# nanless/universal-speech-enhancement

Measured on AMD Instinct MI355X. Metric: spectrogram-frames/sec through 30-step PC sampler, 24 kHz, higher is better.
Workload: dtype bf16; 1 GPU; configs[1]: NCSN++ Large score net, batch=8x4 s utterances per GPU, 30-step PC sampler (reverse_diffusion + langevin x1, snr 0.5, 60 NFE), bf16, hipGraph=on; global_batch=8, frames_per_utt=601, padded_frames_per_utt=640, n_freq=512, N=30, nfe=60, parallelism=utterance-sharded x1

## Files before the change

universal_speech_enhancement_amd/csrc/use_conv_v2.hip:

```cpp
#include "use_kernels.h"
#include "use_device.h"

#include <cstdio>
#include <cstdlib>

namespace use {

constexpr int V2_T = 16;
constexpr int V2_HE = V2_T + 2;
constexpr int V2_HALO = V2_HE * V2_HE;
constexpr int V2_BN = 128;

template <typename TIN, bool ACT>
DEVI uint4 v2_transform(const uint4 raw, const unsigned mask, const float (&ca)[16 / sizeof(TIN)],
                        const float (&cb)[16 / sizeof(TIN)]) {
    constexpr int VEC = 16 / sizeof(TIN);
    float v[VEC];
    Vec16<TIN>::load(reinterpret_cast<const TIN*>(&raw), v);
#pragma unroll
    for (int k = 0; k < VEC; ++k) {
        v[k] = fmaf(v[k], ca[k], cb[k]);
        if (ACT) {
            if (sizeof(TIN) == 4) v[k] = v[k] / (1.0f + expf(-v[k]));
            else v[k] = v[k] * __builtin_amdgcn_rcpf(1.0f + __builtin_amdgcn_exp2f(v[k] * -1.44269504088896341f));
        }
    }
    uint4 o = Vec16<TIN>::pack(v);
    o.x &= mask; o.y &= mask; o.z &= mask; o.w &= mask;
    return o;
}

template <typename TIN, typename TOUT, int CK, bool ACT>
__global__ __launch_bounds__(512) void conv_v2_kernel(ConvArgs p) {
    typedef Mfma<TIN> MF;
    constexpr int VEC = 16 / sizeof(TIN);
    constexpr int PARTS = CK / VEC;
    constexpr int ROWB = CK * (int)sizeof(TIN) + 16;
    constexpr int BN = V2_BN, WM = 4, WN = 2, MW = 64, NW = 64, TM = 2, TN = 2;
    constexpr int KSTEPS = CK / MF::KM;
    constexpr int HPITCH = (V2_HE * ROWB / 16 + 15) / 16 * 16 * 16;
    constexpr int HALO_BYTES = V2_HE * HPITCH, W_BYTES = BN * ROWB;
    constexpr int MAIN_BYTES = 2 * HALO_BYTES + 2 * W_BYTES;
    constexpr int NPIECE = V2_HALO * PARTS;
    constexpr int PIECE_ITERS = (NPIECE + 511) / 512;
    static_assert(PARTS == 8 && 512 % PARTS == 0 && PIECE_ITERS <= 8, "v2 staging assumes 128-byte chunk rows");

    extern __shared__ __attribute__((aligned(16))) char smem[];
    const int tid = threadIdx.x, lane = tid & 63, wave = tid >> 6;
    const int wm = wave / WN, wn = wave % WN;
    const int b = blockIdx.z;
    int tile = blockIdx.x;
    if ((gridDim.x & 7) == 0) tile = (blockIdx.x & 7) * (gridDim.x >> 3) + (blockIdx.x >> 3);
    const int tiles_x = (p.W + V2_T - 1) / V2_T;
    const int ty0 = (tile / tiles_x) * V2_T, tx0 = (tile % tiles_x) * V2_T;
    const int n0 = blockIdx.y * BN;
    const int Ctot = p.C0 + p.C1;
    const int nchunks = Ctot / CK;
    const int XCtot = p.XC0 + p.XC1;
    const int nchunks2 = XCtot / CK;
    const int part = tid & (PARTS - 1);

    float addv[2];
#pragma unroll
    for (int j = 0; j < 2; ++j) {
        const int co = n0 + wn * 64 + j * 32 + (lane & 31);
        float add = 0.f;
// ... 35 lines not shown
    for (int i = 0; i < TM; ++i) {
        const int m = wm * MW + i * 32 + (lane & 31);
        a_base[i] = (m >> 4) * HPITCH + (m & 15) * ROWB + (lane >> 5) * MF::KPL * (int)sizeof(TIN);
    }
#pragma unroll
    for (int j = 0; j < TN; ++j)
        b_base[j] = 2 * HALO_BYTES + (wn * NW + j * 32 + (lane & 31)) * ROWB + (lane >> 5) * MF::KPL * (int)sizeof(TIN);

    int ppix[PIECE_ITERS], pdst[PIECE_ITERS]; unsigned pmask[PIECE_ITERS];
#pragma unroll
    for (int j = 0; j < PIECE_ITERS; ++j) {
        const int idx = j * 512 + tid;
        const int pix = idx / PARTS;
        const int hy = pix / V2_HE, hx = pix - hy * V2_HE;
        const int gy = ty0 + hy - 1, gx = tx0 + hx - 1;
        const bool inb = idx < NPIECE && gy >= 0 && gy < p.H && gx >= 0 && gx < p.W;
        ppix[j] = inb ? gy * p.W + gx : 0;
        pmask[j] = inb ? 0xffffffffu : 0u;
        pdst[j] = idx < NPIECE ? hy * HPITCH + hx * ROWB + part * 16 : -1;
    }
    const int dummy_off = MAIN_BYTES + tid * 16;
    constexpr int COEF_OFF = MAIN_BYTES + 512 * 16;
    float2* const coef_lds = reinterpret_cast<float2*>(smem + COEF_OFF);
    float ca[VEC], cb[VEC];
    auto load_coef = [&](int chunk) {
        const float2* cf = coef_lds + chunk * CK + part * VEC;
#pragma unroll
        for (int k = 0; k < VEC; ++k) { const float2 v = cf[k]; ca[k] = v.x; cb[k] = v.y; }
    };
    auto buf_ld = [&](const void* base, unsigned voff, unsigned soff) -> uint4 {
        const __amdgpu_buffer_rsrc_t rs = __builtin_amdgcn_make_buffer_rsrc(const_cast<void*>(base), 0, 0x7fffffff, 0x00020000);
        return __builtin_bit_cast(uint4, __builtin_amdgcn_raw_buffer_load_b128(rs, voff, soff, 0));
    };
    auto src_ld0 = [&](int chunk, int pixoff) -> uint4 {
        const int c_glob = chunk * CK;
        const TIN* src; int Cs, c_loc;
        if (c_glob < p.C0) { src = (const TIN*)p.src0; Cs = p.C0; c_loc = c_glob; }
        else               { src = (const TIN*)p.src1; Cs = p.C1; c_loc = c_glob - p.C0; }
        const unsigned voff = (unsigned)pixoff * (unsigned)(Cs * (int)sizeof(TIN)) + (unsigned)(part * 16);
        return buf_ld(src + (size_t)b * p.H * p.W * Cs, voff, (unsigned)(c_loc * (int)sizeof(TIN)));
    };
    auto load_piece1 = [&](int chunk2, int q, uint4& raw) -> unsigned {
        const int pix = (q * 512 + tid) / PARTS;
        const int gy = ty0 + (pix >> 4), gx = tx0 + (pix & 15);
        const bool inb = gy < p.H && gx < p.W;
        const int c_glob = chunk2 * CK;
        const TIN* src; int Cs, c_loc;
        if (c_glob < p.XC0) { src = (const TIN*)p.x0; Cs = p.XC0; c_loc = c_glob; }
        else                { src = (const TIN*)p.x1; Cs = p.XC1; c_loc = c_glob - p.XC0; }
        const size_t pixoff = inb ? (size_t)(b * p.H + gy) * p.W + gx : 0;
        raw = *reinterpret_cast<const uint4*>(src + pixoff * Cs + c_loc + part * VEC);
        return inb ? 0xffffffffu : 0u;
    };
    auto piece1_dst = [&](int q, int hb) -> int {
        const int pix = (q * 512 + tid) / PARTS;
        return hb * HALO_BYTES + ((pix >> 4) + 1) * HPITCH + ((pix & 15) + 1) * ROWB + part * 16;
    };

    const int wrow0 = tid / PARTS, wrow1 = (tid + 512) / PARTS;
    const unsigned wo0 = wrow0 * 9 * Ctot + part * VEC, wo1 = wrow1 * 9 * Ctot + part * VEC;
    const unsigned wob0 = wo0 * (unsigned)sizeof(TIN), wob1 = wo1 * (unsigned)sizeof(TIN);
    const int wdst0 = 2 * HALO_BYTES + wrow0 * ROWB + part * 16, wdst1 = 2 * HALO_BYTES + wrow1 * ROWB + part * 16;
    const TIN* const wseg0 = (const TIN*)p.w + (size_t)n0 * 9 * Ctot;
#define V2_LOAD_W(CC, TT, R0, R1)                                                                                    \
    {                                                                                                                \
        const int cw_ = (TT) > 8 ? (CC) + 1 : (CC);                                                                  \
        const int tw_ = (TT) > 8 ? (TT)-9 : (TT);                                                                    \
        if (cw_ < nchunks) {                                                                                         \
            const unsigned so_ = (unsigned)(tw_ * Ctot + cw_ * CK) * (unsigned)sizeof(TIN);                          \
            R0 = buf_ld(wseg0, wob0, so_); R1 = buf_ld(wseg0, wob1, so_);                                            \
        }                                                                                                            \
    }
#define V2_STORE_W(BUF, R0, R1)                                                                     \
    {                                                                                               \
        *reinterpret_cast<uint4*>(smem + (BUF)*W_BYTES + wdst0) = R0;                               \
        *reinterpret_cast<uint4*>(smem + (BUF)*W_BYTES + wdst1) = R1;                               \
    }

    uint4 wa0 = make_uint4(0, 0, 0, 0), wa1 = wa0;
    {
        uint4 w00 = wa0, w01 = wa0, raw[PIECE_ITERS];
        V2_LOAD_W(0, 0, w00, w01);
        V2_LOAD_W(0, 1, wa0, wa1);
#pragma unroll
        for (int j = 0; j < PIECE_ITERS; ++j) raw[j] = src_ld0(0, ppix[j]);
        gn_fill_table(coef_lds, p, b, Ctot, tid, 512);
        __syncthreads();
        load_coef(0);
        V2_STORE_W(0, w00, w01);
#pragma unroll
        for (int j = 0; j < PIECE_ITERS; ++j)
            *reinterpret_cast<uint4*>(smem + (pdst[j] >= 0 ? pdst[j] : dummy_off)) = v2_transform<TIN, ACT>(raw[j], pmask[j], ca, cb);
    }

    V2_STAMP(2)
    typename MF::frag af[KSTEPS][TM], bf[KSTEPS][TN];
    uint4 hL = wa0, hT = wa0, t0 = wa0;
#define V2_LDS(CC, T)                                                                                                \
    {                                                                                                                \
        const int cc_ = (CC);                                                                                        \
        const int par_ = cc_ & 1;                             \
        const bool next_ = cc_ + 1 < nchunks;                                                                        \
        V2_STAMPF(100 + (T))                                                                                          \
        {                                                                                                            \
            const char* ha_ = smem + par_ * HALO_BYTES + ((T) / 3) * HPITCH + ((T) % 3) * ROWB;                      \
            const char* wbuf_ = smem + (par_ ^ ((T)&1)) * W_BYTES;                                                   \
            _Pragma("unroll") for (int kk = 0; kk < KSTEPS; ++kk) {                                                  \
                _Pragma("unroll") for (int i = 0; i < TM; ++i) af[kk][i] = MF::ld(ha_ + a_base[i] + kk * MF::KM * (int)sizeof(TIN)); \
                _Pragma("unroll") for (int j = 0; j < TN; ++j) bf[kk][j] = MF::ld(wbuf_ + b_base[j] + kk * MF::KM * (int)sizeof(TIN)); \
            }                                                                                                        \
        }                                                                                                            \
        __builtin_amdgcn_sched_barrier(0);                                                                           \
        V2_STAMPF(500 + (T))                                                                                          \
        if ((T) >= 2 && (T) < PIECE_ITERS + 2 && next_) {                                                            \
            constexpr int k_ = (T) >= 2 && (T) < PIECE_ITERS + 2 ? (T)-2 : 0;                                        \
            *reinterpret_cast<uint4*>(smem + (pdst[k_] >= 0 ? (par_ ^ 1) * HALO_BYTES + pdst[k_] : dummy_off)) = t0;  \
        }                                                                                                            \
        if ((T) < 8 || next_) V2_STORE_W((par_ ^ ((T)&1)) ^ 1, wa0, wa1);                                            \
        V2_STAMPF(600 + (T))                                                                                          \
        if ((T) >= 1 && (T) < PIECE_ITERS + 1) {                                                                     \
             \
             \
            hT = hL;                                                                                                 \
            asm volatile("" : "+v"(hT.x), "+v"(hT.y), "+v"(hT.z), "+v"(hT.w));                                       \
        }                                                                                                            \
        if ((T) < PIECE_ITERS && next_) {                                                                            \
            if ((T) == 0) load_coef(cc_ + 1);                                                                        \
            constexpr int k_ = (T) < PIECE_ITERS ? (T) : 0;                                                          \
            hL = src_ld0(cc_ + 1, ppix[k_]);                                                                           \
        }                                                                                                            \
        V2_LOAD_W(cc_, (T) + 2, wa0, wa1);                                                                           \
        V2_STAMPF(200 + (T))                                                                                          \
    }
#define V2_MFMA(CC, T)                                                                                               \
    {                                                                                                                \
        V2_STAMPF(300 + (T))                                                                                          \
        _Pragma("unroll") for (int kk = 0; kk < KSTEPS; ++kk)                                                        \
            _Pragma("unroll") for (int i = 0; i < TM; ++i)                                                           \
                _Pragma("unroll") for (int j = 0; j < TN; ++j) acc[i][j] = MF::mma(af[kk][i], bf[kk][j], acc[i][j]);  \
        if ((T) >= 1 && (T) < PIECE_ITERS + 1) {              \
            constexpr int k_ = (T) >= 1 && (T) < PIECE_ITERS + 1 ? (T)-1 : 0;                                        \
            t0 = v2_transform<TIN, ACT>(hT, pmask[k_], ca, cb);                                                      \
            asm volatile("" : "+v"(t0.x), "+v"(t0.y), "+v"(t0.z), "+v"(t0.w));    \
            _Pragma("unroll") for (int g = 0; g < TM * TN * KSTEPS; ++g) {                                           \
                __builtin_amdgcn_sched_group_barrier(0x008, 1, 0);                                      \
                __builtin_amdgcn_sched_group_barrier(0x002, 3, 0);                                      \
                __builtin_amdgcn_sched_group_barrier(0x400, 1, 0);                                      \
            }                                                                                                        \
        }                                                                                                            \
        V2_STAMPF(400 + (T))                                                                                          \
    }

#define V2_BAR() { __builtin_amdgcn_sched_barrier(0); __syncthreads(); __builtin_amdgcn_sched_barrier(0); }
    V2_BAR();
    if (wave < 4) {
        V2_LDS(0, 0)
        V2_BAR();
        for (int c = 0; c < nchunks; ++c) {
#define V2_G0_STEP(T) V2_MFMA(c, T) V2_BAR(); V2_LDS(c, (T) + 1) V2_BAR();
            V2_G0_STEP(0) V2_G0_STEP(1) V2_G0_STEP(2) V2_G0_STEP(3) V2_G0_STEP(4) V2_G0_STEP(5) V2_G0_STEP(6) V2_G0_STEP(7)
#undef V2_G0_STEP
            V2_MFMA(c, 8)
            V2_BAR();
            if (c + 1 < nchunks) V2_LDS(c + 1, 0)
            V2_BAR();
        }
    } else {
        V2_BAR();
        for (int c = 0; c < nchunks; ++c) {
#define V2_G1_STEP(T) V2_LDS(c, T) V2_BAR(); V2_MFMA(c, T) V2_BAR();
            V2_G1_STEP(0) V2_G1_STEP(1) V2_G1_STEP(2) V2_G1_STEP(3) V2_G1_STEP(4) V2_G1_STEP(5) V2_G1_STEP(6) V2_G1_STEP(7) V2_G1_STEP(8)
#undef V2_G1_STEP
        }
    }
#undef V2_BAR
#undef V2_LDS
#undef V2_LOAD_W

    V2_STAMP(3)
    if (nchunks2 > 0) {
        uint4 r0, r1, r2, r3; unsigned m0, m1, m2, m3;
#define V2_SC_LOAD(C2)                                                                                        \
        {                                                                                                     \
            m0 = load_piece1(C2, 0, r0); m1 = load_piece1(C2, 1, r1); m2 = load_piece1(C2, 2, r2); m3 = load_piece1(C2, 3, r3); \
            const TIN* wb_ = (const TIN*)p.w2 + (size_t)n0 * XCtot + (C2)*CK;                                 \
            wa0 = *reinterpret_cast<const uint4*>(wb_ + wrow0 * XCtot + part * VEC);                          \
            wa1 = *reinterpret_cast<const uint4*>(wb_ + wrow1 * XCtot + part * VEC);                          \
        }
        V2_SC_LOAD(0)
        for (int c2 = 0; c2 < nchunks2; ++c2) {
            const int buf = c2 & 1;
            r0.x &= m0; r0.y &= m0; r0.z &= m0; r0.w &= m0; r1.x &= m1; r1.y &= m1; r1.z &= m1; r1.w &= m1;
            r2.x &= m2; r2.y &= m2; r2.z &= m2; r2.w &= m2; r3.x &= m3; r3.y &= m3; r3.z &= m3; r3.w &= m3;
            *reinterpret_cast<uint4*>(smem + piece1_dst(0, buf)) = r0; *reinterpret_cast<uint4*>(smem + piece1_dst(1, buf)) = r1;
            *reinterpret_cast<uint4*>(smem + piece1_dst(2, buf)) = r2; *reinterpret_cast<uint4*>(smem + piece1_dst(3, buf)) = r3;
            V2_STORE_W(buf, wa0, wa1);
            __syncthreads();
            if (c2 + 1 < nchunks2) V2_SC_LOAD(c2 + 1)
            const char* ha_ = smem + buf * HALO_BYTES + HPITCH + ROWB;
            const char* wb2_ = smem + buf * W_BYTES;
#pragma unroll
            for (int kk = 0; kk < KSTEPS; ++kk) {
#pragma unroll
                for (int i = 0; i < TM; ++i) af[kk][i] = MF::ld(ha_ + a_base[i] + kk * MF::KM * (int)sizeof(TIN));
#pragma unroll
                for (int j = 0; j < TN; ++j) bf[kk][j] = MF::ld(wb2_ + b_base[j] + kk * MF::KM * (int)sizeof(TIN));
            }
            V2_MFMA(nchunks, 0)
        }
#undef V2_SC_LOAD
        __syncthreads();
    }
#undef V2_MFMA
#undef V2_STORE_W

    V2_STAMP(4)
    constexpr int STG_LD = NW + 4;
    constexpr int STG_WAVE = 32 * STG_LD * 4;
    constexpr int CH = 16 / (int)sizeof(TOUT);
    constexpr int CPR = NW / CH;
    constexpr int QN = 32 * CPR / 64;
    constexpr int PPP = 64 / CPR;
    float* const stg = reinterpret_cast<float*>(smem + wave * STG_WAVE);
    float* const red = reinterpret_cast<float*>(smem + 8 * STG_WAVE);
    const int ch = lane % CPR, lx = lane / CPR;
    const int co0 = n0 + wn * NW + ch * CH;
    const bool cok = co0 < p.Cout;
    const int wm_u = __builtin_amdgcn_readfirstlane(wm);
    const size_t img_elems = (size_t)p.H * p.W * p.Cout;
    const __amdgpu_buffer_rsrc_t rs_out = __builtin_amdgcn_make_buffer_rsrc((TOUT*)p.out + (size_t)b * img_elems, 0, 0x7fffffff, 0x00020000);
    const __amdgpu_buffer_rsrc_t rs_res = __builtin_amdgcn_make_buffer_rsrc(const_cast<TOUT*>((const TOUT*)p.res) + (size_t)b * img_elems, 0, 0x7fffffff, 0x00020000);
    const unsigned voff = (unsigned)((lx * p.Cout + co0) * (int)sizeof(TOUT));
    const bool has_res = p.res != nullptr, has_scale = p.out_scale != 1.f;
    constexpr bool HOIST_W4 = sizeof(TOUT) == 2;
    float4 w4r[CH]; float b4r[CH];
    if (HOIST_W4 && p.pyr && cok) {
#pragma unroll
        for (int c = 0; c < CH; ++c) { w4r[c] = *reinterpret_cast<const float4*>(p.w4 + (size_t)(co0 + c) * 4); b4r[c] = p.b4[co0 + c]; }
    } else {
#pragma unroll
        for (int c = 0; c < CH; ++c) { w4r[c] = make_float4(0.f, 0.f, 0.f, 0.f); b4r[c] = 0.f; }
    }
    float st_s[CH], st_q[CH];
#pragma unroll
    for (int c = 0; c < CH; ++c) { st_s[c] = 0.f; st_q[c] = 0.f; }
#define V2_EPI_POS(I, Q)                                                                                             \
// ... 54 lines not shown
            if (ok) {
                const uint4 packed = Vec16<TOUT>::pack(v);
                __builtin_amdgcn_raw_buffer_store_b128(__builtin_bit_cast(__attribute__((ext_vector_type(4))) unsigned, packed), rs_out, off, 0, 0);
#pragma unroll
                for (int c = 0; c < CH; ++c) { st_s[c] += v[c]; st_q[c] = fmaf(v[c], v[c], st_q[c]); }
            }
        }
        __builtin_amdgcn_wave_barrier();
        V2_STAMP(42 + 2 * i)
    }
#undef V2_EPI_POS
    if (p.stats) {
#pragma unroll
        for (int c = 0; c < CH; ++c) { st_s[c] = reduce_lanes_stride<CPR>(st_s[c]); st_q[c] = reduce_lanes_stride<CPR>(st_q[c]); }
        if (lane < CPR) {
#pragma unroll
            for (int c = 0; c < CH; ++c) {
                const int cl = wn * NW + ch * CH + c;
                red[(wm * BN + cl) * 2] = st_s[c]; red[(wm * BN + cl) * 2 + 1] = st_q[c];
            }
        }
        __syncthreads();
        if (tid < BN) {
            float s = 0.f, q = 0.f;
#pragma unroll
            for (int w = 0; w < WM; ++w) { s += red[(w * BN + tid) * 2]; q += red[(w * BN + tid) * 2 + 1]; }
            const int co = n0 + tid;
            if (co < p.Cout) gn_accumulate(p.stats + ((size_t)b * p.Cout + co) * 2, s, q);
        }
    }
    V2_STAMP(5)
}

template <typename TIN, typename TOUT, int CK, bool ACT>
static void v2_launch_t(const ConvArgs& a, hipStream_t s) {
    constexpr int ROWB = CK * (int)sizeof(TIN) + 16;
    constexpr int HPITCH = (V2_HE * ROWB / 16 + 15) / 16 * 16 * 16;
    constexpr int MAIN = 2 * V2_HE * HPITCH + 2 * V2_BN * ROWB + 512 * 16 + 1024 * 8;
    constexpr int EPI = 8 * 32 * (64 + 4) * 4 + 4 * V2_BN * 2 * 4;
    constexpr int SMEM = MAIN > EPI ? MAIN : EPI;
    static LdsAttrOnce attr;
    auto kern = conv_v2_kernel<TIN, TOUT, CK, ACT>;
    attr(kern, SMEM);
    dim3 grid(conv_v2_tiles(a.H, a.W), (a.Cout + V2_BN - 1) / V2_BN, a.B);
    hipLaunchKernelGGL(kern, grid, dim3(512), SMEM, s, a);
}

bool conv_v2_eligible(const ConvDesc& a) {
    const int Ctot = a.C0 + a.C1, XC = a.XC0 + a.XC1;
    const int ck = a.in_dtype == DT_F32 ? 32 : 64;
    return a.ntaps == 9 && a.Cout > 32 && a.in_dtype == a.out_dtype && Ctot % ck == 0 && Ctot <= 1024 && XC % ck == 0 &&
           (a.C1 == 0 || a.C0 % ck == 0) && (a.XC1 == 0 || a.XC0 % ck == 0) &&
           a.H >= V2_T && a.W >= V2_T;
}

void launch_conv_v2(const ConvArgs& a0, hipStream_t s) {
    ConvArgs a = a0;
    static const int dbg = getenv("USE_HIP_DBG") ? atoi(getenv("USE_HIP_DBG")) : 0;
    a.dbg = dbg;
    static unsigned long long* trace_buf = nullptr;
    if (getenv("USE_HIP_TRACE")) {
        static int printed = 0;
        const int want_c = atoi(getenv("USE_HIP_TRACE"));
        if (!trace_buf) { (void)hipMalloc((void**)&trace_buf, 512 * 8); }
        if (!printed && a.H == 512 && a.C0 + a.C1 == want_c) {
            (void)hipMemsetAsync(trace_buf, 0, 512 * 8, s);
            a.trace = trace_buf;
            if (a.in_dtype == DT_BF16) { a.act ? v2_launch_t<__bf16, __bf16, 64, true>(a, s) : v2_launch_t<__bf16, __bf16, 64, false>(a, s); }
            (void)hipStreamSynchronize(s);
            unsigned long long hbuf[512];
            (void)hipMemcpy(hbuf, trace_buf, sizeof hbuf, hipMemcpyDeviceToHost);
            for (int g = 0; g < 2; ++g) {
                unsigned long long prev = hbuf[g * 256 + 1];
                for (int i = 0; i < 120 && hbuf[g * 256 + 2 * i]; ++i) {
                    fprintf(stderr, "[trace G%d] id %3llu  +%6llu\n", g, hbuf[g * 256 + 2 * i], hbuf[g * 256 + 2 * i + 1] - prev);
                    prev = hbuf[g * 256 + 2 * i + 1];
                }
            }
            printed = 1;
            a.trace = nullptr;
        }
    }
    if (a.in_dtype == DT_BF16)     { a.act ? v2_launch_t<__bf16, __bf16, 64, true>(a, s) : v2_launch_t<__bf16, __bf16, 64, false>(a, s); }
    else if (a.in_dtype == DT_F16) { a.act ? v2_launch_t<_Float16, _Float16, 64, true>(a, s) : v2_launch_t<_Float16, _Float16, 64, false>(a, s); }
    else                           { a.act ? v2_launch_t<float, float, 32, true>(a, s) : v2_launch_t<float, float, 32, false>(a, s); }
}

}
```

universal_speech_enhancement_amd/csrc/use_device.h:

```cpp
#pragma once
#include <hip/hip_runtime.h>
#include <math.h>
#include <utility>

namespace use {

typedef __attribute__((ext_vector_type(8))) __bf16 bf16x8;
typedef __attribute__((ext_vector_type(8))) _Float16 f16x8;
typedef __attribute__((ext_vector_type(16))) float f32x16;
typedef __attribute__((ext_vector_type(4))) float f32x4;

#define DEVI __device__ __forceinline__

template <bool ACCURATE>
DEVI float silu_f(float x) {
    if (ACCURATE) return x / (1.0f + expf(-x));
    return x * __builtin_amdgcn_rcpf(1.0f + __builtin_amdgcn_exp2f(x * -1.44269504088896341f));
}

typedef float f32x2 __attribute__((ext_vector_type(2)));
template <int N, bool ACT = true>
DEVI void affine_silu_pk(const float (&x)[N], const float (&ca)[N], const float (&cb)[N], float (&y)[N]) {
    static_assert(N % 2 == 0, "pairs of channels");
#pragma unroll
// ... 123 lines not shown
                             : "+v"(c0), "+v"(c1), "+v"(c2), "+v"(d), "=&v"(xl), "=&v"(xh), "=&v"(ul), "=&v"(uh)                         \
                             : "v"(a0), "v"(a1), "v"(a2), "v"(b0), "v"(b1), "v"(b2), "v"(al), "v"(bl), "v"(ah), "v"(bh));               \
            else                                                                                                         \
                asm volatile(MFMA " %0, %8, %11, %0\n\t"                                                                 \
                             LO("%4", "%3") "\n\t" HI("%5", "%3") "\n\tv_fma_f32 %6, %4, %14, %15\n\tv_fma_f32 %7, %5, %16, %17\n\t" \
                             MFMA " %1, %9, %12, %1\n\t"                                                                 \
                             MFMA " %2, %10, %13, %2\n\t" PK("%3", "%6", "%7")                                           \
                             : "+v"(c0), "+v"(c1), "+v"(c2), "+v"(d), "=&v"(xl), "=&v"(xh), "=&v"(ul), "=&v"(uh)                         \
                             : "v"(a0), "v"(a1), "v"(a2), "v"(b0), "v"(b1), "v"(b2), "v"(al), "v"(bl), "v"(ah), "v"(bh));               \
        }                                                                                                                \
    };
#define USE_XF_BF16_LO(D, S) "v_lshlrev_b32 " D ", 16, " S
#define USE_XF_BF16_HI(D, S) "v_and_b32 " D ", 0xffff0000, " S
#define USE_XF_BF16_PK(D, A, B) "v_cvt_pk_bf16_f32 " D ", " A ", " B
#define USE_XF_F16_LO(D, S) "v_cvt_f32_f16 " D ", " S
#define USE_XF_F16_HI(D, S) "v_cvt_f32_f16_sdwa " D ", " S " dst_sel:DWORD dst_unused:UNUSED_PAD src0_sel:WORD_1"
#define USE_XF_F16_PK(D, A, B) "v_cvt_pk_f16_f32 " D ", " A ", " B
USE_XF_ASM_STRINGS(__bf16, "v_mfma_f32_32x32x16_bf16", USE_XF_BF16_LO, USE_XF_BF16_HI, USE_XF_BF16_PK)
USE_XF_ASM_STRINGS(_Float16, "v_mfma_f32_32x32x16_f16", USE_XF_F16_LO, USE_XF_F16_HI, USE_XF_F16_PK)
#undef USE_XF_ASM_STRINGS

template <typename TIN, bool ACT, typename ACC, typename AF, typename BF>
DEVI uint4 mfma16_with_transform(ACC& acc, const AF& af, const BF& bf, const uint4 raw, const float (&ca)[8], const float (&cb)[8]) {
    typedef XfAsm<TIN> X;
    unsigned d[4] = {raw.x, raw.y, raw.z, raw.w};
    X::bare4(acc[0][0], acc[0][1], acc[0][2], acc[0][3], af[0][0], bf[0][0], bf[0][1], bf[0][2], bf[0][3]);
    X::template dword3<ACT>(acc[1][0], acc[1][1], acc[1][2], af[0][1], af[0][1], af[0][1], bf[0][0], bf[0][1], bf[0][2], d[0], ca[0], cb[0], ca[1], cb[1]);
    X::template dword3<ACT>(acc[1][3], acc[0][0], acc[0][1], af[0][1], af[1][0], af[1][0], bf[0][3], bf[1][0], bf[1][1], d[1], ca[2], cb[2], ca[3], cb[3]);
    X::template dword3<ACT>(acc[0][2], acc[0][3], acc[1][0], af[1][0], af[1][0], af[1][1], bf[1][2], bf[1][3], bf[1][0], d[2], ca[4], cb[4], ca[5], cb[5]);
    X::template dword3<ACT>(acc[1][1], acc[1][2], acc[1][3], af[1][1], af[1][1], af[1][1], bf[1][1], bf[1][2], bf[1][3], d[3], ca[6], cb[6], ca[7], cb[7]);
    return make_uint4(d[0], d[1], d[2], d[3]);
}

constexpr int v4_stg_off(int r, int j) { return (j * 512 + r * 64 + 4 * ((j & 1) + 8 * (j >> 1))) * 4; }
constexpr int V4_STG_ATID_BYTES = 8384;
template <int J, int R0, typename ACC>
DEVI void v4_stage8(unsigned lds_base, const ACC& a) {
    unsigned keep;
    asm volatile("s_mov_b32 %[keep], m0\n\ts_mov_b32 m0, %[base]\n\ts_nop 0\n\t"
                 "ds_write_addtid_b32 %[a0] offset:%[o0]\n\tds_write_addtid_b32 %[a1] offset:%[o1]\n\tds_write_addtid_b32 %[a2] offset:%[o2]\n\t"
                 "ds_write_addtid_b32 %[a3] offset:%[o3]\n\tds_write_addtid_b32 %[a4] offset:%[o4]\n\tds_write_addtid_b32 %[a5] offset:%[o5]\n\t"
                 "ds_write_addtid_b32 %[a6] offset:%[o6]\n\tds_write_addtid_b32 %[a7] offset:%[o7]\n\t"
                 "s_mov_b32 m0, %[keep]"
                 : [keep] "=&s"(keep)
                 : [base] "s"(lds_base), [a0] "v"(a[R0]), [a1] "v"(a[R0 + 1]), [a2] "v"(a[R0 + 2]), [a3] "v"(a[R0 + 3]), [a4] "v"(a[R0 + 4]),
                   [a5] "v"(a[R0 + 5]), [a6] "v"(a[R0 + 6]), [a7] "v"(a[R0 + 7]),
                   [o0] "n"(v4_stg_off(0, J)), [o1] "n"(v4_stg_off(1, J)), [o2] "n"(v4_stg_off(2, J)), [o3] "n"(v4_stg_off(3, J)),
                   [o4] "n"(v4_stg_off(4, J)), [o5] "n"(v4_stg_off(5, J)), [o6] "n"(v4_stg_off(6, J)), [o7] "n"(v4_stg_off(7, J))
                 : "memory");
}

constexpr float GN_SUM_SCALE = 1048576.0f, GN_SQ_SCALE = 1048576.0f;
DEVI void gn_accumulate(long long* dst, float s, float q) {
    atomicAdd(reinterpret_cast<unsigned long long*>(dst), (unsigned long long)__float2ll_rn(s * GN_SUM_SCALE));
    atomicAdd(reinterpret_cast<unsigned long long*>(dst + 1), (unsigned long long)__float2ll_rn(q * GN_SQ_SCALE));
}
DEVI float2 gn_coef_of(const long long* __restrict__ st0, int C0, const long long* __restrict__ st1, int C1,
                       const float* __restrict__ gamma, const float* __restrict__ beta, int groups, float inv_n, float eps,
                       int b, int c) {
    const int cpg = (C0 + C1) / groups, g0 = (c / cpg) * cpg;
    long long S = 0, Q = 0;
    for (int k = 0; k < cpg; ++k) {
        const int cc = g0 + k;
        const long long* p = cc < C0 ? st0 + ((size_t)b * C0 + cc) * 2 : st1 + ((size_t)b * C1 + (cc - C0)) * 2;
        S += p[0]; Q += p[1];
    }
// ... 38 lines not shown
```

universal_speech_enhancement_amd/csrc/use_engine.cpp:

```cpp
#include "../../include/use_hip.h"
#include "use_kernels.h"

#include <hip/hip_runtime.h>

#include <algorithm>
#include <cmath>
#include <cstdarg>
#include <cstdio>
#include <cstdlib>
#include <cstring>
#include <map>
#include <memory>
#include <mutex>
#include <string>
#include <unordered_map>
#include <vector>

using namespace use;

static thread_local std::string g_err;
static int fail(int code, const char* fmt, ...) {
    char buf[1024];
    va_list ap; va_start(ap, fmt); vsnprintf(buf, sizeof buf, fmt, ap); va_end(ap);
    g_err = buf;
// ... 1006 lines not shown
    if (!h->cap_stream) HIPCHK(hipStreamCreateWithFlags(&h->cap_stream, hipStreamNonBlocking));
    return USE_OK;
}

extern "C" {

int use_get_stat(use_handle* h, const char* name, long long* value) {
    if (!h || !name || !value) return fail(USE_E_INVALID, "null argument");
    if (!strcmp(name, "graph_captures")) { *value = h->n_graph_captures; return USE_OK; }
    if (!strcmp(name, "plans_built")) { *value = h->n_plans_built; return USE_OK; }
    if (!strcmp(name, "plan_cache_hits")) { *value = h->n_plan_cache_hits; return USE_OK; }
    if (!strcmp(name, "plans_parked")) { *value = (long long)h->parked.size(); return USE_OK; }
    if (!strcmp(name, "ode_steps")) { *value = h->ode_steps; return USE_OK; }
    if (!strcmp(name, "ode_rejected")) { *value = h->ode_rejected; return USE_OK; }
    if (!strcmp(name, "ode_nfev_max")) { *value = h->ode_nfev_max; return USE_OK; }
    if (!strcmp(name, "plan_stale")) { *value = h->plan && h->plan->opt_gen != g_opt_gen ? 1 : 0; return USE_OK; }
    return fail(USE_E_INVALID, "unknown statistic '%s'", name);
}

int use_set_option(const char* name, long long value) {
    if (!name) return fail(USE_E_INVALID, "option name is null");
    if (!strcmp(name, "trace")) { g_trace = value != 0; return USE_OK; }
    if (!strcmp(name, "sampler_trace")) { g_sampler_trace = value != 0; return USE_OK; }
    ++g_opt_gen;
    if (!strcmp(name, "attn_fused")) { g_attn_fused = (int)value; return USE_OK; }
    if (!strcmp(name, "plan_cache")) { g_plan_cache = (int)std::max(0LL, std::min(16LL, value)); return USE_OK; }
    if (!strcmp(name, "subbatch_min_items")) { g_subbatch_min_items = (int)std::max(1LL, value); return USE_OK; }
    if (!strcmp(name, "subbatch")) { g_subbatch = (int)value; return USE_OK; }
    if (!strcmp(name, "stagger_level")) { g_stagger_level = (int)value; return USE_OK; }
    if (!strcmp(name, "stats_part")) { g_stats_part = (int)value; return USE_OK; }
    if (!strcmp(name, "gn_inline")) { g_gn_inline = (long)value; return USE_OK; }
    if (!strcmp(name, "conv_v4_min_blocks")) { conv_v4_set_min_blocks((long)value); return USE_OK; }
    if (!strcmp(name, "conv_v5")) { conv_v5_set((int)value); return USE_OK; }
    if (!strcmp(name, "fir_strip")) { fir_set_strip((int)value); return USE_OK; }
    if (!strcmp(name, "pyr_ws")) { pyr_conv_set_ws((int)value); return USE_OK; }
    if (!strcmp(name, "wgrad_mfma16")) { wgrad_set_mfma16((int)value); return USE_OK; }
    if (!strcmp(name, "wgrad_blocks")) { wgrad_set_blocks((int)value); return USE_OK; }
    if (!strcmp(name, "conv_in_wgs")) { if (value < 1 || value > 4096) return fail(USE_E_INVALID, "conv_in_wgs: 1 ... 4096"); g_conv_in_wgs = (int)value; return USE_OK; }
    if (!strcmp(name, "conv_sk_max_px")) { conv_sk_set_max_px((long)value); return USE_OK; }
    return fail(USE_E_INVALID, "unknown option '%s'", name);
}
const char* use_last_error(void) { return g_err.c_str(); }
const char* use_version(void) { return "use_hip 0.1 (gfx950)"; }

int use_create(const use_config* cfg, int device, use_handle** out) {
    if (!cfg || !out) return fail(USE_E_INVALID, "null argument");
    if (cfg->n_levels < 1 || cfg->n_levels > 8 || cfg->nf % 32 != 0 || cfg->nf < 32 || cfg->num_res_blocks < 1)
        return fail(USE_E_INVALID, "unsupported architecture (nf must be a multiple of 32, 1..8 levels)");
    for (int i = 0; i < cfg->n_levels; ++i)
        if (cfg->ch_mult[i] < 1 || cfg->nf * cfg->ch_mult[i] > 512) return fail(USE_E_INVALID, "unsupported architecture (1 <= nf * ch_mult <= 512)");
    if (cfg->n_freq % (1 << (cfg->n_levels - 1)) != 0)
        return fail(USE_E_INVALID, "n_freq=%d is not divisible by 2^(levels-1)", cfg->n_freq);
    if (cfg->precision != USE_PREC_FP32 && cfg->precision != USE_PREC_BF16 && cfg->precision != USE_PREC_FP16) return fail(USE_E_INVALID, "bad precision");
    if (cfg->input_channels != 0 && cfg->input_channels != 2 && cfg->input_channels != 4 && cfg->input_channels != 6)
        return fail(USE_E_INVALID, "input_channels must be 4 (x and y), 6 (x, y and a second conditioning) or 2 (y alone), got %d", cfg->input_channels);
    use_handle* h = new use_handle();
    h->cfg = *cfg; h->device = device;
    h->act_dtype = cfg->precision == USE_PREC_BF16 ? DT_BF16 : cfg->precision == USE_PREC_FP16 ? DT_F16 : DT_F32;
    int rc = build_arch(h);
    if (rc) { delete h; return rc; }
    *out = h;
    return USE_OK;
}

int use_destroy(use_handle* h) {
    if (!h) return USE_OK;
// ... 1589 lines not shown
```

universal_speech_enhancement_amd/csrc/use_kernels.h:

```cpp
#pragma once
#include <hip/hip_runtime.h>
#include <stdint.h>
#include <atomic>
#include <thread>

namespace use {

constexpr int USE_MAX_DEVICES = 64;
struct LdsAttrOnce {
    std::atomic<int> st[USE_MAX_DEVICES] = {};
    template <typename F> void once(F&& f) {
        int d = 0;
        if (hipGetDevice(&d) != hipSuccess || d < 0 || d >= USE_MAX_DEVICES) { f(); return; }
        if (st[d].load(std::memory_order_acquire) == 2) return;
        int expected = 0;
        if (st[d].compare_exchange_strong(expected, 1, std::memory_order_acq_rel)) { f(); st[d].store(2, std::memory_order_release); }
        else while (st[d].load(std::memory_order_acquire) != 2) std::this_thread::yield();
    }
    template <typename K> void operator()(K kern, int bytes) {
        once([&] { (void)hipFuncSetAttribute(reinterpret_cast<const void*>(kern), hipFuncAttributeMaxDynamicSharedMemorySize, bytes); });
    }
};


// ... 45 lines not shown
    ConvDesc d{};
    d.H = a.H; d.W = a.W; d.C0 = a.C0; d.C1 = a.C1; d.XC0 = a.XC0; d.XC1 = a.XC1; d.Cout = a.Cout; d.cout_pad = a.cout_pad; d.ntaps = a.ntaps;
    d.in_dtype = a.in_dtype; d.out_dtype = a.out_dtype; d.act = a.act;
    d.coef = a.coef != nullptr; d.w = a.w != nullptr; d.wb = a.wb != nullptr; d.w2 = a.w2 != nullptr; d.w2b = a.w2b != nullptr;
    d.res = a.res != nullptr; d.pyr = a.pyr != nullptr; d.temb = a.temb != nullptr; d.stats = a.stats != nullptr || a.stats_part != nullptr;
    return d;
}
enum ConvKernel { SK, WIDE32, WIDE16, V2, PYR, PYR_WS, IN, IN_SPLIT, GENERIC };
struct ConvChoice {
    ConvKernel k;
    int stats_parts;
    const char* label;
    bool hbm;
};
ConvChoice conv_choose(const ConvDesc& d);
const char* conv_kernel_name(ConvKernel k);
void launch_conv(const ConvArgs& a, hipStream_t s);
int launch_conv_variant(const ConvArgs& a, int variant, hipStream_t s, const char** why);
bool conv_v2_eligible(const ConvDesc& d);
void launch_conv_v2(const ConvArgs& a, hipStream_t s);
inline int conv_v4_chunk(int dtype) { return dtype == DT_F32 ? 16 : 32; }
inline int conv_v4_tiles(int H, int W) { return ((H + 15) / 16) * ((W + 31) / 32); }
bool conv_sk_eligible(const ConvDesc& d);
void conv_sk_set_max_px(long n);
void launch_conv_sk(const ConvArgs& a, hipStream_t s);
void conv_sk_set_per_image(bool on);
void pyr_conv_set_ws(int n);
bool conv_v4_eligible(const ConvDesc& d);
const char* conv_v4_unrunnable(const ConvDesc& d);
void conv_v4_set_min_blocks(long n);
void launch_conv_v4(const ConvArgs& a, hipStream_t s);
const char* conv_v5_unrunnable(const ConvDesc& d);
void conv_v5_set(int on);
bool conv_v5_enabled(const ConvDesc& d);
void launch_conv_v5(const ConvArgs& a, hipStream_t s);
void launch_gn_finalize(const long long* st0, int C0, const long long* st1, int C1, const float* gamma, const float* beta,
                        int groups, int hw, float eps, float* coef, int B, hipStream_t s, const long long* pt0 = nullptr, int nt0 = 0,
                        const long long* pt1 = nullptr, int nt1 = 0);

void launch_fir_up2(const void* src, int dtype, const float* coef, int act, void* out_act, void* out_raw, int B,
                    int H, int W, int C, hipStream_t s);
void fir_set_strip(int on);
void launch_fir_down2(const void* src, int dtype, const float* coef, int act, void* out_act, void* out_raw, int B,
                      int H, int W, int C, hipStream_t s);

void launch_spec_map(const float2* in, float2* out, long rows, int Tin, int Tin_stride, int Tout, float pre, float power,
                     float post, hipStream_t s);

void launch_chunk_split(const float2* Y, float2* chunks, int B, int F, int n, int Tp, int C, int overlap, hipStream_t s);
void launch_chunk_merge(const float2* chunks, float2* X, int B, int F, int n, int Tp, int C, int overlap, hipStream_t s);

void launch_item_lengths(int* lens, const int* len_host, int B, hipStream_t s);
constexpr int METRICS_SLICE = 2048;
struct MetricsWork { size_t part1, part2, alpha, lsd, bytes; int nblk, Tmax; };
MetricsWork metrics_layout(int B, int stride);
void launch_metrics(const float* est, const float* clean, const float* noise, const int* len_host, int B, int stride, void* work,
                    double* out, hipStream_t s);

void launch_twiddle_table(float2* tw, int N, hipStream_t s);
void launch_stft_fwd(const float* wav, const float* win, const float2* tw, float2* Y, int B, int L, int N, int hop, int T,
                     int Tpad, float factor, float expo, hipStream_t s);
void launch_istft_back(const float2* X, const float* win, const float2* tw, float* wav, int B, int L, int N, int hop, int Tpad,
                       float factor, float expo, hipStream_t s);
void launch_stft_fwd_items(const float* wav, long stride, const int* len_host, const float* win, const float2* tw, float2* Y, int B,
                           int N, int hop, int Tpad, float factor, float expo, hipStream_t s);
void launch_istft_back_items(const float2* X, const float* win, const float2* tw, float* wav, long stride, const int* len_host, int B,
// ... 104 lines not shown
```

Baseline: 3665 spectrogram-frames/s.

## Interleave halo GroupNorm/SiLU transform with MFMA in conv_v2 main loop

Adds a SCHED variant of the v2 3x3 conv kernel, on by default for 16-bit types. It interleaves the next chunk's halo load and GroupNorm+SiLU transform with the MFMA issue through a helper that mixes transform instructions between MFMAs. Branches on chunk bounds become unconditional buffer loads, using a zero-range resource descriptor for dead chunks. Out-of-bounds halo pixels are zeroed once up front, so the per-piece mask is dropped. The aim is to hide transform ALU work and load latency under the matrix ops, at the cost of more register pressure and a more fragile hand schedule.

```diff
diff --git a/universal_speech_enhancement_amd/csrc/use_conv_v2.hip b/universal_speech_enhancement_amd/csrc/use_conv_v2.hip
--- a/universal_speech_enhancement_amd/csrc/use_conv_v2.hip
+++ b/universal_speech_enhancement_amd/csrc/use_conv_v2.hip
@@ -30,8 +30,9 @@
     return o;
 }
 
-template <typename TIN, typename TOUT, int CK, bool ACT>
+template <typename TIN, typename TOUT, int CK, bool ACT, bool SCHED>
 __global__ __launch_bounds__(512) void conv_v2_kernel(ConvArgs p) {
+    static_assert(!SCHED || (sizeof(TIN) == 2 && sizeof(TOUT) == 2), "SCHED: 16-bit storage");
     typedef Mfma<TIN> MF;
     constexpr int VEC = 16 / sizeof(TIN);
     constexpr int PARTS = CK / VEC;
@@ -133,6 +134,19 @@
         const __amdgpu_buffer_rsrc_t rs = __builtin_amdgcn_make_buffer_rsrc(const_cast<void*>(base), 0, 0x7fffffff, 0x00020000);
         return __builtin_bit_cast(uint4, __builtin_amdgcn_raw_buffer_load_b128(rs, voff, soff, 0));
     };
+    auto buf_ld_live = [&](const void* base, unsigned voff, unsigned soff, int live) -> uint4 {
+        const __amdgpu_buffer_rsrc_t rs = __builtin_amdgcn_make_buffer_rsrc(const_cast<void*>(base), 0, live ? 0x7fffffff : 0, 0x00020000);
+        return __builtin_bit_cast(uint4, __builtin_amdgcn_raw_buffer_load_b128(rs, voff, soff, 0));
+    };
+    auto src_ld0_live = [&](int chunk0, int pixoff) -> uint4 {
+        const int chunk = chunk0 < nchunks ? chunk0 : nchunks - 1;
+        const int c_glob = chunk * CK;
+        const TIN* src; int Cs, c_loc;
+        if (c_glob < p.C0) { src = (const TIN*)p.src0; Cs = p.C0; c_loc = c_glob; }
+        else               { src = (const TIN*)p.src1; Cs = p.C1; c_loc = c_glob - p.C0; }
+        const unsigned voff = (unsigned)pixoff * (unsigned)(Cs * (int)sizeof(TIN)) + (unsigned)(part * 16);
+        return buf_ld_live(src + (size_t)b * p.H * p.W * Cs, voff, (unsigned)(c_loc * (int)sizeof(TIN)), chunk0 < nchunks);
+    };
     auto src_ld0 = [&](int chunk, int pixoff) -> uint4 {
         const int c_glob = chunk * CK;
         const TIN* src; int Cs, c_loc;
@@ -167,7 +181,11 @@
     {                                                                                                                \
         const int cw_ = (TT) > 8 ? (CC) + 1 : (CC);                                                                  \
         const int tw_ = (TT) > 8 ? (TT)-9 : (TT);                                                                    \
-        if (cw_ < nchunks) {                                                                                         \
+        if constexpr (SCHED) {                                              \
+            const int cl_ = cw_ < nchunks ? cw_ : nchunks - 1;                                                       \
+            const unsigned so_ = (unsigned)(tw_ * Ctot + cl_ * CK) * (unsigned)sizeof(TIN);                          \
+            R0 = buf_ld_live(wseg0, wob0, so_, cw_ < nchunks); R1 = buf_ld_live(wseg0, wob1, so_, cw_ < nchunks);    \
+        } else if (cw_ < nchunks) {                                                                                  \
             const unsigned so_ = (unsigned)(tw_ * Ctot + cw_ * CK) * (unsigned)sizeof(TIN);                          \
             R0 = buf_ld(wseg0, wob0, so_); R1 = buf_ld(wseg0, wob1, so_);                                            \
         }                                                                                                            \
@@ -185,19 +203,30 @@
         V2_LOAD_W(0, 1, wa0, wa1);
 #pragma unroll
         for (int j = 0; j < PIECE_ITERS; ++j) raw[j] = src_ld0(0, ppix[j]);
+        if constexpr (SCHED) {
+            __builtin_amdgcn_sched_barrier(0);
+#pragma unroll
+            for (int j = 0; j < PIECE_ITERS; ++j) {
+                if (pdst[j] >= 0 && pmask[j] == 0u) {
+                    *reinterpret_cast<uint4*>(smem + pdst[j]) = make_uint4(0, 0, 0, 0);
+                    *reinterpret_cast<uint4*>(smem + HALO_BYTES + pdst[j]) = make_uint4(0, 0, 0, 0);
+                }
+                if (pmask[j] == 0u) pdst[j] = -1;
+            }
+        }
         gn_fill_table(coef_lds, p, b, Ctot, tid, 512);
         __syncthreads();
         load_coef(0);
         V2_STORE_W(0, w00, w01);
 #pragma unroll
         for (int j = 0; j < PIECE_ITERS; ++j)
-            *reinterpret_cast<uint4*>(smem + (pdst[j] >= 0 ? pdst[j] : dummy_off)) = v2_transform<TIN, ACT>(raw[j], pmask[j], ca, cb);
+            *reinterpret_cast<uint4*>(smem + (pdst[j] >= 0 ? pdst[j] : dummy_off)) = v2_transform<TIN, ACT>(raw[j], SCHED ? 0xffffffffu : pmask[j], ca, cb);
     }
 
     V2_STAMP(2)
     typename MF::frag af[KSTEPS][TM], bf[KSTEPS][TN];
     uint4 hL = wa0, hT = wa0, t0 = wa0;
-#define V2_LDS(CC, T)                                                                                                \
+#define V2_LDS_L(CC, T)                                                                                              \
     {                                                                                                                \
         const int cc_ = (CC);                                                                                        \
         const int par_ = cc_ & 1;                             \
@@ -233,7 +262,7 @@
         V2_LOAD_W(cc_, (T) + 2, wa0, wa1);                                                                           \
         V2_STAMPF(200 + (T))                                                                                          \
     }
-#define V2_MFMA(CC, T)                                                                                               \
+#define V2_MFMA_L(CC, T)                                                                                             \
     {                                                                                                                \
         V2_STAMPF(300 + (T))                                                                                          \
         _Pragma("unroll") for (int kk = 0; kk < KSTEPS; ++kk)                                                        \
@@ -251,6 +280,45 @@
         }                                                                                                            \
         V2_STAMPF(400 + (T))                                                                                          \
     }
+    uint4 hN[2] = {wa0, wa0};
+#define V2_LDS_N(CC, T)                                                                                              \
+    {                                                                                                                \
+        const int cc_ = (CC);                                                                                        \
+        const int par_ = cc_ & 1;                                                                                    \
+        {                                                                                                            \
+            const char* ha_ = smem + par_ * HALO_BYTES + ((T) / 3) * HPITCH + ((T) % 3) * ROWB;                      \
+            const char* wbuf_ = smem + (par_ ^ ((T)&1)) * W_BYTES;                                                   \
+            _Pragma("unroll") for (int kk = 0; kk < KSTEPS; ++kk) {                                                  \
+                _Pragma("unroll") for (int i = 0; i < TM; ++i) af[kk][i] = MF::ld(ha_ + a_base[i] + kk * MF::KM * (int)sizeof(TIN)); \
+                _Pragma("unroll") for (int j = 0; j < TN; ++j) bf[kk][j] = MF::ld(wbuf_ + b_base[j] + kk * MF::KM * (int)sizeof(TIN)); \
+            }                                                                                                        \
+        }                                                                                                            \
+        __builtin_amdgcn_sched_barrier(0);                                                                           \
+        if ((T) >= 2 && (T) < PIECE_ITERS + 2) {                                                                     \
+            constexpr int k_ = (T) >= 2 && (T) < PIECE_ITERS + 2 ? (T)-2 : 0;                                        \
+            *reinterpret_cast<uint4*>(smem + (pdst[k_] >= 0 ? (par_ ^ 1) * HALO_BYTES + pdst[k_] : dummy_off)) = t0;  \
+        }                                                                                                            \
+        V2_STORE_W((par_ ^ ((T)&1)) ^ 1, wa0, wa1);                                                                  \
+        V2_LOAD_W(cc_, (T) + 2, wa0, wa1);                                                                           \
+        if ((T) < PIECE_ITERS) {                                                                                     \
+            if ((T) == 0) load_coef(cc_ + 1 < nchunks ? cc_ + 1 : nchunks - 1);                                      \
+            constexpr int k_ = (T) < PIECE_ITERS ? (T) : 0;                                                          \
+            hN[k_ & 1] = src_ld0_live(cc_ + 1, ppix[k_]);                                                            \
+        }                                                                                                            \
+    }
+#define V2_MFMA_N(CC, T)                                                                                             \
+    {                                                                                                                \
+        if ((T) >= 1 && (T) < PIECE_ITERS + 1) {                                                                     \
+            constexpr int k_ = (T) >= 1 && (T) < PIECE_ITERS + 1 ? (T)-1 : 0;                                        \
+            t0 = mfma16_2x2x4_with_transform<TIN, ACT>(acc, af, bf, hN[k_ & 1], ca, cb);                             \
+        } else {                                                                                                     \
+            _Pragma("unroll") for (int kk = 0; kk < KSTEPS; ++kk)                                                    \
+                _Pragma("unroll") for (int i = 0; i < TM; ++i)                                                       \
+                    _Pragma("unroll") for (int j = 0; j < TN; ++j) acc[i][j] = MF::mma(af[kk][i], bf[kk][j], acc[i][j]); \
+        }                                                                                                            \
+    }
+#define V2_LDS(CC, T) { if constexpr (SCHED) V2_LDS_N(CC, T) else V2_LDS_L(CC, T) }
+#define V2_MFMA(CC, T) { if constexpr (SCHED) V2_MFMA_N(CC, T) else V2_MFMA_L(CC, T) }
 
 #define V2_BAR() { __builtin_amdgcn_sched_barrier(0); __syncthreads(); __builtin_amdgcn_sched_barrier(0); }
     V2_BAR();
@@ -263,7 +331,7 @@
 #undef V2_G0_STEP
             V2_MFMA(c, 8)
             V2_BAR();
-            if (c + 1 < nchunks) V2_LDS(c + 1, 0)
+            if (SCHED || c + 1 < nchunks) V2_LDS(c + 1, 0)
             V2_BAR();
         }
     } else {
@@ -276,6 +344,8 @@
     }
 #undef V2_BAR
 #undef V2_LDS
+#undef V2_LDS_L
+#undef V2_LDS_N
 #undef V2_LOAD_W
 
     V2_STAMP(3)
@@ -313,6 +383,8 @@
         __syncthreads();
     }
 #undef V2_MFMA
+#undef V2_MFMA_L
+#undef V2_MFMA_N
 #undef V2_STORE_W
 
     V2_STAMP(4)
@@ -433,7 +505,7 @@
     V2_STAMP(5)
 }
 
-template <typename TIN, typename TOUT, int CK, bool ACT>
+template <typename TIN, typename TOUT, int CK, bool ACT, bool SCHED>
 static void v2_launch_t(const ConvArgs& a, hipStream_t s) {
     constexpr int ROWB = CK * (int)sizeof(TIN) + 16;
     constexpr int HPITCH = (V2_HE * ROWB / 16 + 15) / 16 * 16 * 16;
@@ -441,7 +513,7 @@
     constexpr int EPI = 8 * 32 * (64 + 4) * 4 + 4 * V2_BN * 2 * 4;
     constexpr int SMEM = MAIN > EPI ? MAIN : EPI;
     static LdsAttrOnce attr;
-    auto kern = conv_v2_kernel<TIN, TOUT, CK, ACT>;
+    auto kern = conv_v2_kernel<TIN, TOUT, CK, ACT, SCHED>;
     attr(kern, SMEM);
     dim3 grid(conv_v2_tiles(a.H, a.W), (a.Cout + V2_BN - 1) / V2_BN, a.B);
     hipLaunchKernelGGL(kern, grid, dim3(512), SMEM, s, a);
@@ -453,6 +525,15 @@
     return a.ntaps == 9 && a.Cout > 32 && a.in_dtype == a.out_dtype && Ctot % ck == 0 && Ctot <= 1024 && XC % ck == 0 &&
            (a.C1 == 0 || a.C0 % ck == 0) && (a.XC1 == 0 || a.XC0 % ck == 0) &&
            a.H >= V2_T && a.W >= V2_T;
+}
+
+static int g_conv_v2_sched = 1;
+void conv_v2_sched_set(int on) { g_conv_v2_sched = on; }
+
+template <typename T>
+static void v2_launch16(const ConvArgs& a, hipStream_t s) {
+    if (g_conv_v2_sched) { a.act ? v2_launch_t<T, T, 64, true, true>(a, s) : v2_launch_t<T, T, 64, false, true>(a, s); }
+    else                 { a.act ? v2_launch_t<T, T, 64, true, false>(a, s) : v2_launch_t<T, T, 64, false, false>(a, s); }
 }
 
 void launch_conv_v2(const ConvArgs& a0, hipStream_t s) {
@@ -467,7 +548,7 @@
         if (!printed && a.H == 512 && a.C0 + a.C1 == want_c) {
             (void)hipMemsetAsync(trace_buf, 0, 512 * 8, s);
             a.trace = trace_buf;
-            if (a.in_dtype == DT_BF16) { a.act ? v2_launch_t<__bf16, __bf16, 64, true>(a, s) : v2_launch_t<__bf16, __bf16, 64, false>(a, s); }
+            if (a.in_dtype == DT_BF16) v2_launch16<__bf16>(a, s);
             (void)hipStreamSynchronize(s);
             unsigned long long hbuf[512];
             (void)hipMemcpy(hbuf, trace_buf, sizeof hbuf, hipMemcpyDeviceToHost);
@@ -482,9 +563,9 @@
             a.trace = nullptr;
         }
     }
-    if (a.in_dtype == DT_BF16)     { a.act ? v2_launch_t<__bf16, __bf16, 64, true>(a, s) : v2_launch_t<__bf16, __bf16, 64, false>(a, s); }
-    else if (a.in_dtype == DT_F16) { a.act ? v2_launch_t<_Float16, _Float16, 64, true>(a, s) : v2_launch_t<_Float16, _Float16, 64, false>(a, s); }
-    else                           { a.act ? v2_launch_t<float, float, 32, true>(a, s) : v2_launch_t<float, float, 32, false>(a, s); }
-}
-
-}
+    if (a.in_dtype == DT_BF16)     v2_launch16<__bf16>(a, s);
+    else if (a.in_dtype == DT_F16) v2_launch16<_Float16>(a, s);
+    else                           { a.act ? v2_launch_t<float, float, 32, true, false>(a, s) : v2_launch_t<float, float, 32, false, false>(a, s); }
+}
+
+}
diff --git a/universal_speech_enhancement_amd/csrc/use_device.h b/universal_speech_enhancement_amd/csrc/use_device.h
--- a/universal_speech_enhancement_amd/csrc/use_device.h
+++ b/universal_speech_enhancement_amd/csrc/use_device.h
@@ -179,6 +179,22 @@
     return make_uint4(d[0], d[1], d[2], d[3]);
 }
 
+template <typename TIN, bool ACT, typename ACC, typename AF, typename BF>
+DEVI uint4 mfma16_2x2x4_with_transform(ACC& acc, const AF& af, const BF& bf, const uint4 raw, const float (&ca)[8], const float (&cb)[8]) {
+    typedef XfAsm<TIN> X;
+    typedef Mfma<TIN> MF;
+    unsigned d[4] = {raw.x, raw.y, raw.z, raw.w};
+#pragma unroll
+    for (int i = 0; i < 2; ++i)
+#pragma unroll
+        for (int j = 0; j < 2; ++j) acc[i][j] = MF::mma(af[0][i], bf[0][j], acc[i][j]);
+    X::template dword3<ACT>(acc[0][0], acc[0][1], acc[1][0], af[1][0], af[1][0], af[1][1], bf[1][0], bf[1][1], bf[1][0], d[0], ca[0], cb[0], ca[1], cb[1]);
+    X::template dword3<ACT>(acc[1][1], acc[0][0], acc[0][1], af[1][1], af[2][0], af[2][0], bf[1][1], bf[2][0], bf[2][1], d[1], ca[2], cb[2], ca[3], cb[3]);
+    X::template dword3<ACT>(acc[1][0], acc[1][1], acc[0][0], af[2][1], af[2][1], af[3][0], bf[2][0], bf[2][1], bf[3][0], d[2], ca[4], cb[4], ca[5], cb[5]);
+    X::template dword3<ACT>(acc[0][1], acc[1][0], acc[1][1], af[3][0], af[3][1], af[3][1], bf[3][1], bf[3][0], bf[3][1], d[3], ca[6], cb[6], ca[7], cb[7]);
+    return make_uint4(d[0], d[1], d[2], d[3]);
+}
+
 constexpr int v4_stg_off(int r, int j) { return (j * 512 + r * 64 + 4 * ((j & 1) + 8 * (j >> 1))) * 4; }
 constexpr int V4_STG_ATID_BYTES = 8384;
 template <int J, int R0, typename ACC>
diff --git a/universal_speech_enhancement_amd/csrc/use_engine.cpp b/universal_speech_enhancement_amd/csrc/use_engine.cpp
--- a/universal_speech_enhancement_amd/csrc/use_engine.cpp
+++ b/universal_speech_enhancement_amd/csrc/use_engine.cpp
@@ -1062,6 +1062,7 @@
     if (!strcmp(name, "gn_inline")) { g_gn_inline = (long)value; return USE_OK; }
     if (!strcmp(name, "conv_v4_min_blocks")) { conv_v4_set_min_blocks((long)value); return USE_OK; }
     if (!strcmp(name, "conv_v5")) { conv_v5_set((int)value); return USE_OK; }
+    if (!strcmp(name, "conv_v2_sched")) { conv_v2_sched_set((int)value); return USE_OK; }
     if (!strcmp(name, "fir_strip")) { fir_set_strip((int)value); return USE_OK; }
     if (!strcmp(name, "pyr_ws")) { pyr_conv_set_ws((int)value); return USE_OK; }
     if (!strcmp(name, "wgrad_mfma16")) { wgrad_set_mfma16((int)value); return USE_OK; }
diff --git a/universal_speech_enhancement_amd/csrc/use_kernels.h b/universal_speech_enhancement_amd/csrc/use_kernels.h
--- a/universal_speech_enhancement_amd/csrc/use_kernels.h
+++ b/universal_speech_enhancement_amd/csrc/use_kernels.h
@@ -101,6 +101,7 @@
 void launch_conv_v4(const ConvArgs& a, hipStream_t s);
 const char* conv_v5_unrunnable(const ConvDesc& d);
 void conv_v5_set(int on);
+void conv_v2_sched_set(int on);
 bool conv_v5_enabled(const ConvDesc& d);
 void launch_conv_v5(const ConvArgs& a, hipStream_t s);
 void launch_gn_finalize(const long long* st0, int C0, const long long* st1, int C1, const float* gamma, const float* beta,
```

Result: no change. 3669 spectrogram-frames/s, median of 6 (+0.1%).
